# hzxie/RMNet

Hardware: AMD Instinct MI355X
Metric: frames/sec at 480p, 1 object, T=5 memory; memory-read HBM GB/s vs peak (higher is better)
Workload: dtype f32 convs; memory read = fp16 operands (K, V, q, P rounded to 11 bits), fp32 accumulate (RMNET_BANK_F16): the frame loop's default for clips with one object -- on one-object 480x854 clips whose masks HAVE a boundary (tests/live_fixture.py) mask IoU vs the CPU path 0.99993-0.99997 and foreground logi

## Files before the change

### include/rmnet_hip.h

```cpp
#ifndef RMNET_HIP_H_
#define RMNET_HIP_H_

#include <stddef.h>
#include <stdint.h>

#ifdef __cplusplus
extern "C" {
#endif

#define RMNET_ABI_VERSION 6

enum {
  RMNET_OK = 0,
  RMNET_E_INVALID_ARG = -1,
  RMNET_E_WORKSPACE = -2,
  RMNET_E_LAUNCH = -3,
  RMNET_E_UNSUPPORTED = -4
};

int rmnet_abi_version(void);
const char *rmnet_error_string(int code);

size_t rmnet_region_map_workspace_bytes(int B, int K, int H, int W);
int rmnet_region_map_f32(const float *mask, int B, int K, int H, int W, float prob_threshold,
                         int n_pts_threshold, int n_bbox_loose_pixels, float *att_map,
                         int32_t *bboxes, int32_t *cell_rects, int pad_l, int pad_t,
                         int cell_stride, int cells_h, int cells_w, void *workspace,
                         size_t workspace_bytes, void *stream);

int rmnet_region_map_warped_f32(const float *mask, const float *flow, int B, int K, int H, int W,
                                float prob_threshold, int n_pts_threshold, int n_bbox_loose_pixels,
                                float *att_map, int32_t *bboxes, int32_t *cell_rects, int pad_l,
                                int pad_t, int cell_stride, int cells_h, int cells_w, float *warped,
                                void *workspace, size_t workspace_bytes, void *stream);

int rmnet_boxes_to_cell_rects_i32(const int32_t *bboxes, int n_boxes, int k_per_batch, int pad_l,
                                  int pad_t, int cell_stride, int cells_h, int cells_w,
                                  int32_t *cell_rects, void *stream);

#define RMNET_MR_DEFAULT 0
#define RMNET_MR_FORCE_GENERIC 1
#define RMNET_MR_EXACT_FP32 2
#define RMNET_MR_F16 4
#define RMNET_BANK_F16 4
#define RMNET_MR_QX 8
#define RMNET_BANK_QX 8

size_t rmnet_memory_read_workspace_bytes(int no, int De, int Do, int T, int h, int w, int flags);
int rmnet_memory_read_f32(const float *m_key, const float *m_val, const float *q_key,
                          const float *q_val, int no, int De, int Do, int T, int h, int w,
                          long long m_chan_stride, long long m_obj_stride, long long v_chan_stride,
                          long long v_obj_stride, float *mem_val, float *p_out,
                          const int32_t *mem_rects, const int32_t *qry_rects, int flags,
                          void *workspace, size_t workspace_bytes, void *stream);

int rmnet_memory_read_f32_ev(const float *m_key, const float *m_val, const float *q_key,
                             const float *q_val, int no, int De, int Do, int T, int h, int w,
                             long long m_chan_stride, long long m_obj_stride,
                             long long v_chan_stride, long long v_obj_stride, float *mem_val,
                             float *p_out, const int32_t *mem_rects, const int32_t *qry_rects,
                             int flags, void *workspace, size_t workspace_bytes, void *stream,
                             void *ev_start, void *ev_mid, void *ev_end);

size_t rmnet_bank_bytes(int no, int Tcap, int h, int w);
size_t rmnet_bank_overflow_offset(int no, int Tcap, int h, int w);
size_t rmnet_bank_area_offset(int no, int Tcap, int h, int w);
int rmnet_bank_append_f32(void *bank, int no, int Tcap, int h, int w, int slot, const float *k4,
                          const float *v4, const int32_t *rects, void *stream);
int rmnet_bank_append_f32_at(void *bank, int no, int Tcap, int h, int w, int slot, const int32_t *slot_dev,
                             const float *k4, const float *v4, const int32_t *rects, void *stream);
int rmnet_bank_read_f32_at(void *bank, int no, int Tcap, int h, int w, int T, const int32_t *T_dev, int flags,
                           const float *q_key, const float *q_val, const int32_t *qry_rects,
                           float *mem_val, void *workspace, size_t workspace_bytes, void *stream,
                           void *ev_start, void *ev_mid, void *ev_end);
size_t rmnet_bank_read_workspace_bytes(int no, int h, int w);
size_t rmnet_bank_read_workspace_bytes_for(int no, int h, int w, int T);
int rmnet_bank_read_f32(void *bank, int no, int Tcap, int h, int w, int T,
                        const float *q_key, const float *q_val, const int32_t *qry_rects,
                        float *mem_val, void *workspace, size_t workspace_bytes, void *stream,
                        void *ev_start, void *ev_mid, void *ev_end);

int rmnet_rect_mask_f32(const float *x, int n, int C, int T, int h, int w, const int32_t *rects,
                        float *y, void *stream);

int rmnet_channel_affine_f32(const float *x, const float *scale, const float *shift,
                             const float *res, const float *res_scale, const float *res_shift,
                             int relu, long long N, int C, long long HW, float *out, void *stream);

int rmnet_affine_relu_maxpool_f32(const float *x, const float *scale, const float *shift, long long N,
                                  int C, int H, int W, float *out, void *stream);

int rmnet_upsample2x_add_f32(const float *x, const float *skip, long long N, int C, int h, int w,
                             float *out, void *stream);

int rmnet_channel_affine_nhwc_f32(const float *x, const float *scale, const float *shift, const float *res, const float *res_scale,
                                  const float *res_shift, int relu, long long rows, int C, float *out, void *stream);
int rmnet_upsample2x_add_nhwc_f32(const float *x, const float *skip, long long N, int C, int h, int w, float *out, void *stream);
int rmnet_affine_relu_maxpool_nhwc_f32(const float *x, const float *scale, const float *shift, long long N, int C, int H, int W,
                                       float *out, void *stream);

#define RMNET_CONV_RELU_IN 1
#define RMNET_CONV_RELU_OUT 2
int rmnet_conv3x3_split_f32(const float *x, const void *wpack, const float *w_unscale, const float *bias, const float *res, int flags,
                            int N, int H, int W, int Cin, float *out, int32_t *range_word, void *stream);

int rmnet_conv_split_f32(const float *x, const void *wpack, const float *w_unscale, const float *shift, const float *res, int flags,
                         int N, int H, int W, int Cin, int Cout, int ksize, int stride, float *out, float *out2, int out_split,
                         int32_t *range_word, void *stream);

#define RMNET_CONV_X_SPLIT 4
#define RMNET_CONV_OUT_SPLIT 8
int rmnet_conv_split_pre_f32(const void *x, const void *wpack, const float *w_unscale, const float *shift, const float *res, int flags,
                             int N, int H, int W, int Cin, int Cout, int ksize, int stride, void *out, float *out2, int out_split,
                             int32_t *range_word, void *stream);
int rmnet_split_act_f32(const float *x, long long M, int C, int relu, void *out, int32_t *range_word, void *stream);

int rmnet_stem_split_f32(const float *frame, const float *mask, const float *other, const void *wpack, const float *w_unscale,
                         const float *shift, int N, int H, int W, float *out, int32_t *range_word, void *stream);

int rmnet_pred_head_f32(const float *x, const float *w, const float *bias, int n, int Hq, int Wq, int C, float *out, void *stream);

#define RMNET_FLOW_RELU 1
#define RMNET_FLOW_LEAKY 2
#define RMNET_FLOW_TRANSPOSED 4
int rmnet_flow_conv_f32(const float *x, int x_ld, const void *wpack, const float *w_unscale, const float *shift, int flags, int N, int H,
                        int W, int Cin, int Cout, int ksize, int stride, float *out, int out_ld, int coff, int32_t *range_word,
                        void *stream);

size_t rmnet_flow_head_workspace_bytes(int N, int H, int W, int Cin);
int rmnet_flow_head_f32(const float *x, int x_ld, const float *wpack, const float *bias, int N, int H, int W, int Cin, float *out,
                        void *workspace, size_t workspace_bytes, void *stream);

int rmnet_flow_up_f32(const float *flow, const float *w, int N, int h, int w_, float *out, int out_ld, int coff, void *stream);

int rmnet_soft_aggregate_f32(const float *dec, const int32_t *obj_begin, int B, int K, int Hp, int Wp,
                             int pad_l, int pad_t, int H, int W, float *logit, float *prob,
                             void *stream);

int rmnet_flow_affine_f32(const float *flow, const float *m1, const float *m2, int H, int W,
                          float *out, void *stream);
size_t rmnet_flow_affine_workspace_bytes(int H, int W);
int rmnet_flow_affine_f32_host(const float *flow_host, const float *m1_host, const float *m2_host,
                               int H, int W, float *out_host, void *workspace,
                               size_t workspace_bytes, void *stream);

#ifdef __cplusplus
}
#endif
#endif
```

### rmnet_amd/_lib.py

```python

import ctypes
import os

_HERE = os.path.dirname(os.path.abspath(__file__))
LIB_PATH = os.environ.get('RMNET_HIP_LIB') or os.path.join(_HERE, 'librmnet_hip.so')

c_f32p = ctypes.c_void_p
c_i32p = ctypes.c_void_p

SIGNATURES = {
    'rmnet_abi_version': (ctypes.c_int, []),
    'rmnet_error_string': (ctypes.c_char_p, [ctypes.c_int]),
    'rmnet_region_map_workspace_bytes': (ctypes.c_size_t, [ctypes.c_int] * 4),
    'rmnet_region_map_f32': (ctypes.c_int, [
        c_f32p, ctypes.c_int, ctypes.c_int, ctypes.c_int, ctypes.c_int, ctypes.c_float, ctypes.c_int,
        ctypes.c_int, c_f32p, c_i32p, c_i32p, ctypes.c_int, ctypes.c_int, ctypes.c_int, ctypes.c_int,
        ctypes.c_int, ctypes.c_void_p, ctypes.c_size_t, ctypes.c_void_p]),
    'rmnet_region_map_warped_f32': (ctypes.c_int, [
        c_f32p, c_f32p, ctypes.c_int, ctypes.c_int, ctypes.c_int, ctypes.c_int, ctypes.c_float, ctypes.c_int,
        ctypes.c_int, c_f32p, c_i32p, c_i32p, ctypes.c_int, ctypes.c_int, ctypes.c_int, ctypes.c_int,
        ctypes.c_int, c_f32p, ctypes.c_void_p, ctypes.c_size_t, ctypes.c_void_p]),
    'rmnet_boxes_to_cell_rects_i32': (ctypes.c_int, [
        c_i32p, ctypes.c_int, ctypes.c_int, ctypes.c_int, ctypes.c_int, ctypes.c_int, ctypes.c_int,
        ctypes.c_int, c_i32p, ctypes.c_void_p]),
    'rmnet_memory_read_workspace_bytes': (ctypes.c_size_t, [ctypes.c_int] * 7),
    'rmnet_memory_read_f32': (ctypes.c_int, [
        c_f32p, c_f32p, c_f32p, c_f32p, ctypes.c_int, ctypes.c_int, ctypes.c_int, ctypes.c_int,
        ctypes.c_int, ctypes.c_int, ctypes.c_longlong, ctypes.c_longlong, ctypes.c_longlong,
        ctypes.c_longlong, c_f32p, c_f32p, c_i32p, c_i32p, ctypes.c_int, ctypes.c_void_p,
        ctypes.c_size_t, ctypes.c_void_p]),
    'rmnet_memory_read_f32_ev': (ctypes.c_int, [
        c_f32p, c_f32p, c_f32p, c_f32p, ctypes.c_int, ctypes.c_int, ctypes.c_int, ctypes.c_int,
        ctypes.c_int, ctypes.c_int, ctypes.c_longlong, ctypes.c_longlong, ctypes.c_longlong,
        ctypes.c_longlong, c_f32p, c_f32p, c_i32p, c_i32p, ctypes.c_int, ctypes.c_void_p,
        ctypes.c_size_t, ctypes.c_void_p, ctypes.c_void_p, ctypes.c_void_p, ctypes.c_void_p]),
    'rmnet_bank_bytes': (ctypes.c_size_t, [ctypes.c_int] * 4),
    'rmnet_bank_overflow_offset': (ctypes.c_size_t, [ctypes.c_int] * 4),
    'rmnet_bank_area_offset': (ctypes.c_size_t, [ctypes.c_int] * 4),
    'rmnet_bank_append_f32': (ctypes.c_int, [
        ctypes.c_void_p, ctypes.c_int, ctypes.c_int, ctypes.c_int, ctypes.c_int, ctypes.c_int, c_f32p,
        c_f32p, c_i32p, ctypes.c_void_p]),
    'rmnet_bank_append_f32_at': (ctypes.c_int, [
        ctypes.c_void_p, ctypes.c_int, ctypes.c_int, ctypes.c_int, ctypes.c_int, ctypes.c_int, c_i32p, c_f32p,
        c_f32p, c_i32p, ctypes.c_void_p]),
    'rmnet_bank_read_f32_at': (ctypes.c_int, [
        ctypes.c_void_p, ctypes.c_int, ctypes.c_int, ctypes.c_int, ctypes.c_int, ctypes.c_int, c_i32p, ctypes.c_int, c_f32p,
        c_f32p, c_i32p, c_f32p, ctypes.c_void_p, ctypes.c_size_t, ctypes.c_void_p, ctypes.c_void_p,
        ctypes.c_void_p, ctypes.c_void_p]),
    'rmnet_bank_read_workspace_bytes': (ctypes.c_size_t, [ctypes.c_int] * 3),
    'rmnet_bank_read_workspace_bytes_for': (ctypes.c_size_t, [ctypes.c_int] * 4),
    'rmnet_bank_read_f32': (ctypes.c_int, [
        ctypes.c_void_p, ctypes.c_int, ctypes.c_int, ctypes.c_int, ctypes.c_int, ctypes.c_int, c_f32p,
        c_f32p, c_i32p, c_f32p, ctypes.c_void_p, ctypes.c_size_t, ctypes.c_void_p, ctypes.c_void_p,
        ctypes.c_void_p, ctypes.c_void_p]),
    'rmnet_rect_mask_f32': (ctypes.c_int, [
        c_f32p, ctypes.c_int, ctypes.c_int, ctypes.c_int, ctypes.c_int, ctypes.c_int, c_i32p, c_f32p,
        ctypes.c_void_p]),
    'rmnet_channel_affine_f32': (ctypes.c_int, [
        c_f32p, c_f32p, c_f32p, c_f32p, c_f32p, c_f32p, ctypes.c_int, ctypes.c_longlong, ctypes.c_int,
        ctypes.c_longlong, c_f32p, ctypes.c_void_p]),
    'rmnet_upsample2x_add_f32': (ctypes.c_int, [
        c_f32p, c_f32p, ctypes.c_longlong, ctypes.c_int, ctypes.c_int, ctypes.c_int, c_f32p, ctypes.c_void_p]),
    'rmnet_soft_aggregate_f32': (ctypes.c_int, [
        c_f32p, c_i32p, ctypes.c_int, ctypes.c_int, ctypes.c_int, ctypes.c_int, ctypes.c_int, ctypes.c_int,
        ctypes.c_int, ctypes.c_int, c_f32p, c_f32p, ctypes.c_void_p]),
    'rmnet_affine_relu_maxpool_f32': (ctypes.c_int, [
        c_f32p, c_f32p, c_f32p, ctypes.c_longlong, ctypes.c_int, ctypes.c_int, ctypes.c_int, c_f32p,
        ctypes.c_void_p]),
    'rmnet_channel_affine_nhwc_f32': (ctypes.c_int, [
        c_f32p, c_f32p, c_f32p, c_f32p, c_f32p, c_f32p, ctypes.c_int, ctypes.c_longlong, ctypes.c_int, c_f32p, ctypes.c_void_p]),
    'rmnet_upsample2x_add_nhwc_f32': (ctypes.c_int, [
        c_f32p, c_f32p, ctypes.c_longlong, ctypes.c_int, ctypes.c_int, ctypes.c_int, c_f32p, ctypes.c_void_p]),
    'rmnet_affine_relu_maxpool_nhwc_f32': (ctypes.c_int, [
        c_f32p, c_f32p, c_f32p, ctypes.c_longlong, ctypes.c_int, ctypes.c_int, ctypes.c_int, c_f32p, ctypes.c_void_p]),
    'rmnet_conv3x3_split_f32': (ctypes.c_int, [
        c_f32p, ctypes.c_void_p, c_f32p, c_f32p, c_f32p, ctypes.c_int, ctypes.c_int, ctypes.c_int, ctypes.c_int, ctypes.c_int,
        c_f32p, c_i32p, ctypes.c_void_p]),
    'rmnet_conv_split_f32': (ctypes.c_int, [
        c_f32p, ctypes.c_void_p, c_f32p, c_f32p, c_f32p, ctypes.c_int, ctypes.c_int, ctypes.c_int, ctypes.c_int, ctypes.c_int,
        ctypes.c_int, ctypes.c_int, ctypes.c_int, c_f32p, c_f32p, ctypes.c_int, c_i32p, ctypes.c_void_p]),
    'rmnet_conv_split_pre_f32': (ctypes.c_int, [
        ctypes.c_void_p, ctypes.c_void_p, c_f32p, c_f32p, c_f32p, ctypes.c_int, ctypes.c_int, ctypes.c_int, ctypes.c_int, ctypes.c_int,
        ctypes.c_int, ctypes.c_int, ctypes.c_int, ctypes.c_void_p, c_f32p, ctypes.c_int, c_i32p, ctypes.c_void_p]),
    'rmnet_split_act_f32': (ctypes.c_int, [
        c_f32p, ctypes.c_longlong, ctypes.c_int, ctypes.c_int, ctypes.c_void_p, c_i32p, ctypes.c_void_p]),
    'rmnet_stem_split_f32': (ctypes.c_int, [
        c_f32p, c_f32p, c_f32p, ctypes.c_void_p, c_f32p, c_f32p, ctypes.c_int, ctypes.c_int, ctypes.c_int, c_f32p, c_i32p,
        ctypes.c_void_p]),
    'rmnet_pred_head_f32': (ctypes.c_int, [
        c_f32p, c_f32p, c_f32p, ctypes.c_int, ctypes.c_int, ctypes.c_int, ctypes.c_int, c_f32p, ctypes.c_void_p]),
    'rmnet_flow_conv_f32': (ctypes.c_int, [
        c_f32p, ctypes.c_int, ctypes.c_void_p, c_f32p, c_f32p, ctypes.c_int, ctypes.c_int, ctypes.c_int, ctypes.c_int, ctypes.c_int,
        ctypes.c_int, ctypes.c_int, ctypes.c_int, c_f32p, ctypes.c_int, ctypes.c_int, c_i32p, ctypes.c_void_p]),
    'rmnet_flow_head_workspace_bytes': (ctypes.c_size_t, [ctypes.c_int] * 4),
    'rmnet_flow_head_f32': (ctypes.c_int, [
        c_f32p, ctypes.c_int, c_f32p, c_f32p, ctypes.c_int, ctypes.c_int, ctypes.c_int, ctypes.c_int, c_f32p, ctypes.c_void_p,
        ctypes.c_size_t, ctypes.c_void_p]),
    'rmnet_flow_up_f32': (ctypes.c_int, [
        c_f32p, c_f32p, ctypes.c_int, ctypes.c_int, ctypes.c_int, c_f32p, ctypes.c_int, ctypes.c_int, ctypes.c_void_p]),
    'rmnet_flow_affine_f32': (ctypes.c_int, [
        c_f32p, c_f32p, c_f32p, ctypes.c_int, ctypes.c_int, c_f32p, ctypes.c_void_p]),
    'rmnet_flow_affine_workspace_bytes': (ctypes.c_size_t, [ctypes.c_int, ctypes.c_int]),
    'rmnet_flow_affine_f32_host': (ctypes.c_int, [
        ctypes.c_void_p, ctypes.c_void_p, ctypes.c_void_p, ctypes.c_int, ctypes.c_int,
        ctypes.c_void_p, ctypes.c_void_p, ctypes.c_size_t, ctypes.c_void_p]),
}

ABI_VERSION = 6
_lib = None


class RMNetHipError(RuntimeError):
    pass


def load():
    global _lib
    if _lib is not None:
        return _lib
    if not os.path.exists(LIB_PATH):
        raise RMNetHipError(
            'librmnet_hip.so is missing (%s). The HIP kernels are the only implementation of this '
            'path; build them with `python -m rmnet_amd.build`.' % LIB_PATH)
    lib = ctypes.CDLL(LIB_PATH)
    for name, (res, args) in SIGNATURES.items():
        fn = getattr(lib, name)
        fn.restype = res
        fn.argtypes = args
    if lib.rmnet_abi_version() != ABI_VERSION:
        raise RMNetHipError('librmnet_hip.so ABI %d != expected %d' % (lib.rmnet_abi_version(), ABI_VERSION))
    _lib = lib
    return lib


def check(code, what):
    if code != 0:
        msg = load().rmnet_error_string(code).decode()
        raise RMNetHipError('%s failed: %s (code %d)' % (what, msg, code))
```

### rmnet_amd/csrc/conv3x3.hip

```cpp
#include "common.h"

namespace rmnet {
namespace {

typedef _Float16 half8 __attribute__((ext_vector_type(8)));
typedef _Float16 half4 __attribute__((ext_vector_type(4)));
typedef float f32x4 __attribute__((ext_vector_type(4)));
typedef unsigned int u32x4 __attribute__((ext_vector_type(4)));

constexpr int kCout = 256;
constexpr int kMT = 128;
constexpr int kKT = 32;
constexpr int kThreads = 512;
constexpr float kActScale = 64.0f;
constexpr float kActUnscale = 1.0f / 64.0f;
constexpr float kF16Max = 65504.0f;
constexpr int kXPlane = kMT * kKT;
constexpr int kWPlane = kCout * kKT;
constexpr int kBufHalves = 2 * kXPlane + 2 * kWPlane;
static_assert(2 * kBufHalves * 2 <= kLdsBytesPerCU, "LDS budget");

__device__ inline int swz(int row, int chunk) { return row * kKT + ((chunk ^ ((row >> 1) & 3)) << 3); }

template <bool B>
// ... 69 lines not shown
    _Float16* xl = buf + kXPlane;
#pragma unroll
    for (int i = 0; i < 2; ++i) {
      half4 hi, lo;
#pragma unroll
      for (int e = 0; e < 4; ++e) {
        float v = in[i] ? xr[i][e] : 0.0f;
        if constexpr (decltype(relu)::value) v = v < 0.0f ? 0.0f : v;
        const float y = v * kActScale;
        if constexpr (decltype(centre)::value) bad += !(fabsf(y) <= kF16Max) ? 1 : 0;
        const float c = fminf(fmaxf(y, -kF16Max), kF16Max);
        const _Float16 h = (_Float16)c;
        hi[e] = h;
        lo[e] = (_Float16)(c - (float)h);
      }
      const int p = (tid >> 3) + 64 * i;
      const int o = swz(p, c4 >> 1) + 4 * (c4 & 1);
      *reinterpret_cast<half4*>(xh + o) = hi;
      *reinterpret_cast<half4*>(xl + o) = lo;
    }
  };
  auto store_w = [&](_Float16* buf) {
    _Float16* wb = buf + 2 * kXPlane;
#pragma unroll
    for (int i = 0; i < 4; ++i) {
      const int q = tid + kThreads * i;
      const int plane = q >> 10, co = (q >> 2) & (kCout - 1), ch = q & 3;
      *reinterpret_cast<u32x4*>(wb + plane * kWPlane + swz(co, ch)) = wr[i];
    }
  };

  f32x4 acc[4][4], accx[4][4];
#pragma unroll
  for (int i = 0; i < 4; ++i)
#pragma unroll
    for (int j = 0; j < 4; ++j) acc[i][j] = accx[i][j] = f32x4{0.f, 0.f, 0.f, 0.f};

  set_tap(0);
  load();
  if (a.relu_in)
    store_x(Flag<true>{}, Flag<false>{}, lds);
  else
    store_x(Flag<false>{}, Flag<false>{}, lds);
  store_w(lds);
  __syncthreads();
  const int fr = lane & 15, fc = lane >> 4;
  auto mma = [&](const _Float16* __restrict__ cur, auto&& halfway) __attribute__((always_inline)) {
    const _Float16* xh = cur;
    const _Float16* xl = cur + kXPlane;
    const _Float16* wh = cur + 2 * kXPlane;
    const _Float16* wl = wh + kWPlane;
    half8 bh[4], bl[4];
#pragma unroll
    for (int i = 0; i < 4; ++i) {
      const int o = swz(wm * 64 + i * 16 + fr, fc);
      bh[i] = *reinterpret_cast<const half8*>(xh + o);
      bl[i] = *reinterpret_cast<const half8*>(xl + o);
    }
#pragma unroll
    for (int j = 0; j < 4; ++j) {
      const int o = swz(wn * 64 + j * 16 + fr, fc);
      const half8 ah = *reinterpret_cast<const half8*>(wh + o);
      const half8 al = *reinterpret_cast<const half8*>(wl + o);
#pragma unroll
      for (int i = 0; i < 4; ++i) acc[i][j] = __builtin_amdgcn_mfma_f32_16x16x32_f16(ah, bh[i], acc[i][j], 0, 0, 0);
#pragma unroll
      for (int i = 0; i < 4; ++i) accx[i][j] = __builtin_amdgcn_mfma_f32_16x16x32_f16(ah, bl[i], accx[i][j], 0, 0, 0);
#pragma unroll
      for (int i = 0; i < 4; ++i) accx[i][j] = __builtin_amdgcn_mfma_f32_16x16x32_f16(al, bh[i], accx[i][j], 0, 0, 0);
      if (j == 1) halfway();
    }
  };
  int par = 0;
  auto run_taps = [&](auto relu, auto centre, int t0, int t1) __attribute__((always_inline)) {
#pragma unroll 1
    for (int tap = t0; tap < t1; ++tap) {
      if (tap) set_tap(tap);
      const int n = tap ? CB : CB - 1;
      for (int k = 0; k < n; ++k) {
        _Float16* nxt = lds + (par ^ 1) * kBufHalves;
        load();
        __builtin_amdgcn_sched_barrier(0);
        mma(lds + par * kBufHalves, [&] {
          __builtin_amdgcn_sched_barrier(0);
          store_x(relu, centre, nxt);
        });
#pragma unroll
        for (int g = 0; g < 24; ++g) {
          __builtin_amdgcn_sched_group_barrier(0x008, 1, 0);
          __builtin_amdgcn_sched_group_barrier(0x002, 3, 0);
        }
        __builtin_amdgcn_sched_barrier(0);
        store_w(nxt);
        __syncthreads();
        par ^= 1;
      }
    }
  };
  auto run = [&](auto relu) __attribute__((always_inline)) {
    run_taps(relu, Flag<false>{}, 0, 4);
    run_taps(relu, Flag<true>{}, 4, 5);
    run_taps(relu, Flag<false>{}, 5, 9);
  };
  if (a.relu_in)
    run(Flag<true>{});
  else
    run(Flag<false>{});
  mma(lds + par * kBufHalves, [] {});

  f32x4 r[4][4];
  if (a.res) {
#pragma unroll
    for (int i = 0; i < 4; ++i) {
      const int m = m0 + wm * 64 + i * 16 + fr;
#pragma unroll
      for (int j = 0; j < 4; ++j) {
        const int co = wn * 64 + j * 16 + 4 * fc;
        r[i][j] = m < a.M ? *reinterpret_cast<const f32x4*>(a.res + (size_t)m * kCout + co) : f32x4{0.f, 0.f, 0.f, 0.f};
      }
    }
  }
#pragma unroll
  for (int j = 0; j < 4; ++j) {
    const int co = wn * 64 + j * 16 + 4 * fc;
    const f32x4 us = *reinterpret_cast<const f32x4*>(a.w_unscale + co) * kActUnscale;
    const f32x4 b = a.bias ? *reinterpret_cast<const f32x4*>(a.bias + co) : f32x4{0.f, 0.f, 0.f, 0.f};
#pragma unroll
    for (int i = 0; i < 4; ++i) acc[i][j] = (acc[i][j] + accx[i][j]) * us + b;
  }
#pragma unroll
  for (int j = 0; j < 4; ++j)
#pragma unroll
    for (int i = 0; i < 4; ++i) asm volatile("" : "+v"(acc[i][j]));
#pragma unroll
  for (int j = 0; j < 4; ++j) {
    const int co = wn * 64 + j * 16 + 4 * fc;
#pragma unroll
    for (int i = 0; i < 4; ++i) {
      const int m = m0 + wm * 64 + i * 16 + fr;
      if (m >= a.M) continue;
      const size_t off = (size_t)m * kCout + co;
      f32x4 v = acc[i][j];
      if (a.res) v += r[i][j];
      if (a.relu_out) {
#pragma unroll
        for (int e = 0; e < 4; ++e) v[e] = v[e] < 0.0f ? 0.0f : v[e];
      }
      *reinterpret_cast<f32x4*>(a.out + off) = v;
    }
  }
  if (a.range && bad) atomicAdd(a.range, bad);
}

}
}

extern "C" int rmnet_conv3x3_split_f32(const float* x, const void* wpack, const float* w_unscale, const float* bias,
                                       const float* res, int flags, int N, int H, int W, int Cin, float* out,
                                       int32_t* range_word, void* stream) {
  using namespace rmnet;
  if (!x || !wpack || !w_unscale || !out || N <= 0 || H <= 0 || W <= 0 || Cin <= 0) return RMNET_E_INVALID_ARG;
  if (flags & ~(RMNET_CONV_RELU_IN | RMNET_CONV_RELU_OUT)) return RMNET_E_INVALID_ARG;
  if ((reinterpret_cast<uintptr_t>(x) | reinterpret_cast<uintptr_t>(wpack) | reinterpret_cast<uintptr_t>(w_unscale) |
       reinterpret_cast<uintptr_t>(bias) | reinterpret_cast<uintptr_t>(res) | reinterpret_cast<uintptr_t>(out)) & 15)
    return RMNET_E_INVALID_ARG;
  if (Cin % kKT) return RMNET_E_UNSUPPORTED;
  const long long M = (long long)N * H * W;
  if (M * (long long)(Cin > kCout ? Cin : kCout) >= (1LL << 31)) return RMNET_E_UNSUPPORTED;
  const char* xb = reinterpret_cast<const char*>(x);
  const char* ob = reinterpret_cast<const char*>(out);
  if (ob < xb + M * Cin * sizeof(float) && xb < ob + M * kCout * sizeof(float)) return RMNET_E_INVALID_ARG;
  ConvArgs a;
  a.x = x; a.wp = reinterpret_cast<const half8*>(wpack); a.w_unscale = w_unscale; a.bias = bias; a.res = res; a.out = out;
  a.range = range_word; a.M = (int)M; a.H = H; a.W = W; a.Cin = Cin;
  a.relu_in = (flags & RMNET_CONV_RELU_IN) != 0;
  a.relu_out = (flags & RMNET_CONV_RELU_OUT) != 0;
  hipLaunchKernelGGL(conv3x3_split, dim3((unsigned)((M + kMT - 1) / kMT)), dim3(kThreads), 0, (hipStream_t)stream, a);
  return check_launch();
}
```

### rmnet_amd/ops.py

```python

import ctypes

import numpy as np
import torch

from . import _lib


MR_FORCE_GENERIC = 1
MR_EXACT_FP32 = 2
BANK_MAX_SLOTS = 2048


def _check(t, name, dtype=torch.float32):
    if not isinstance(t, torch.Tensor):
        raise RuntimeError('%s must be a torch.Tensor' % name)
    if not t.is_cuda:
        raise RuntimeError('%s must be a CUDA tensor' % name)
    if not t.is_contiguous():
        raise RuntimeError('%s must be contiguous' % name)
    if t.dtype != dtype:
        raise RuntimeError('%s must be %s, got %s' % (name, dtype, t.dtype))


def _is_cl(t):
    return t.dim() == 4 and not t.is_contiguous() and t.is_contiguous(memory_format=torch.channels_last)


def _check_act(t, name):
    if not isinstance(t, torch.Tensor) or not t.is_cuda:
        raise RuntimeError('%s must be a CUDA tensor' % name)
    if t.dtype != torch.float32:
        raise RuntimeError('%s must be torch.float32, got %s' % (name, t.dtype))
    if not (t.is_contiguous() or _is_cl(t)):
        raise RuntimeError('%s must be contiguous (NCHW) or channels-last' % name)


def _stream(dev):
    return ctypes.c_void_p(torch.cuda.current_stream(dev).cuda_stream)


def _ptr(t):
    return ctypes.c_void_p(t.data_ptr()) if t is not None else None


def _ws(nbytes, dev):
    return torch.empty(max(int(nbytes), 256), dtype=torch.uint8, device=dev)


def region_map(mask, prob_threshold=0.5, n_pts_threshold=10, n_bbox_loose_pixels=64,
               want_map=True, cell_grid=None, flow=None, want_warped=False):
    _check(mask, 'mask')
    if mask.dim() != 4:
        raise RuntimeError('mask must be [B, K, H, W]')
    if flow is not None:
        return _region_map_warped(mask, flow, prob_threshold, n_pts_threshold, n_bbox_loose_pixels,
                                  want_map, cell_grid, want_warped)
    if want_warped:
        raise RuntimeError('want_warped needs a flow')
    lib = _lib.load()
    B, K, H, W = mask.shape
    dev = mask.device
    with torch.cuda.device(dev):
        att = torch.empty_like(mask) if want_map else None
        bboxes = torch.empty(B, K, 4, dtype=torch.int32, device=dev)
        rects = torch.empty(B, K, 4, dtype=torch.int32, device=dev) if cell_grid is not None else None
        pl, pt, st, ch, cw = cell_grid if cell_grid is not None else (0, 0, 16, 1, 1)
        nb = lib.rmnet_region_map_workspace_bytes(B, K, H, W)
        ws = _ws(nb, dev)
        rc = lib.rmnet_region_map_f32(_ptr(mask), B, K, H, W, float(prob_threshold),
                                      int(n_pts_threshold), int(n_bbox_loose_pixels), _ptr(att),
                                      _ptr(bboxes), _ptr(rects), int(pl), int(pt), int(st), int(ch),
                                      int(cw), _ptr(ws), ws.numel(), _stream(dev))
    _lib.check(rc, 'rmnet_region_map_f32')
    return att, bboxes, rects


def _region_map_warped(mask, flow, prob_threshold, n_pts_threshold, n_bbox_loose_pixels, want_map,
                       cell_grid, want_warped):
    _check(flow, 'flow')
    B, K, H, W = mask.shape
    if tuple(flow.shape) != (B, 2, H, W):
        raise RuntimeError('flow must be [B, 2, H, W]')
    lib = _lib.load()
    dev = mask.device
    with torch.cuda.device(dev):
        att = torch.empty_like(mask) if want_map else None
        bboxes = torch.empty(B, K, 4, dtype=torch.int32, device=dev)
        rects = torch.empty(B, K, 4, dtype=torch.int32, device=dev) if cell_grid is not None else None
        warped = torch.zeros_like(mask) if want_warped else None
        pl, pt, st, ch, cw = cell_grid if cell_grid is not None else (0, 0, 16, 1, 1)
        nb = lib.rmnet_region_map_workspace_bytes(B, K, H, W)
        ws = _ws(nb, dev)
        rc = lib.rmnet_region_map_warped_f32(_ptr(mask), _ptr(flow), B, K, H, W, float(prob_threshold),
                                             int(n_pts_threshold), int(n_bbox_loose_pixels), _ptr(att),
                                             _ptr(bboxes), _ptr(rects), int(pl), int(pt), int(st),
                                             int(ch), int(cw), _ptr(warped), _ptr(ws), ws.numel(),
                                             _stream(dev))
    _lib.check(rc, 'rmnet_region_map_warped_f32')
    return (att, bboxes, rects, warped) if want_warped else (att, bboxes, rects)


def boxes_to_cell_rects(bboxes, pad_l, pad_t, stride, cells_h, cells_w, k_per_batch=0):
    _check(bboxes, 'bboxes', torch.int32)
    lib = _lib.load()
    dev = bboxes.device
    out = torch.empty_like(bboxes)
    with torch.cuda.device(dev):
        rc = lib.rmnet_boxes_to_cell_rects_i32(_ptr(bboxes), bboxes.numel() // 4, int(k_per_batch),
                                               int(pad_l), int(pad_t), int(stride), int(cells_h),
                                               int(cells_w), _ptr(out), _stream(dev))
    _lib.check(rc, 'rmnet_boxes_to_cell_rects_i32')
    return out


def memory_read(m_key, m_val, q_key, q_val, mem_rects=None, qry_rects=None, want_p=False, flags=0,
                T=None, out=None, events=None):
    for t, n in ((m_key, 'm_key'), (m_val, 'm_val'), (q_key, 'q_key'), (q_val, 'q_val')):
        _check(t, n)
    if m_key.dim() != 5 or m_val.dim() != 5 or q_key.dim() != 4 or q_val.dim() != 4:
        raise RuntimeError('expected m_key/m_val [no,C,T,h,w] and q_key/q_val [no,C,h,w]')
    no, De, Tcap, h, w = m_key.shape
    Do = m_val.shape[1]
    if (m_val.shape[0], m_val.shape[2], m_val.shape[3], m_val.shape[4]) != (no, Tcap, h, w) or \
            tuple(q_key.shape) != (no, De, h, w) or tuple(q_val.shape) != (no, Do, h, w):
        raise RuntimeError('memory/query shapes do not agree')
    T = Tcap if T is None else int(T)
    if not 1 <= T <= Tcap:
        raise RuntimeError('T must be in [1, %d]' % Tcap)
    if (mem_rects is None) != (qry_rects is None):
        raise RuntimeError('mem_rects and qry_rects must be given together')
    if mem_rects is not None:
        _check(mem_rects, 'mem_rects', torch.int32)
        _check(qry_rects, 'qry_rects', torch.int32)
        if mem_rects.numel() != no * T * 4 or qry_rects.numel() != no * 4:
            raise RuntimeError('mem_rects must be [no,T,4] and qry_rects [no,4]')
    lib = _lib.load()
    dev = m_key.device
    with torch.cuda.device(dev):
        if out is None:
            out = torch.empty(no, 2 * Do, h, w, dtype=torch.float32, device=dev)
        else:
            _check(out, 'out')
        p = torch.empty(no, T * h * w, h * w, dtype=torch.float32, device=dev) if want_p else None
        nb = lib.rmnet_memory_read_workspace_bytes(no, De, Do, T, h, w, int(flags))
        ws = _ws(nb, dev)
        cs = Tcap * h * w
        ev = [ctypes.c_void_p(e) if e else None for e in (events or (None, None, None))]
        rc = lib.rmnet_memory_read_f32_ev(_ptr(m_key), _ptr(m_val), _ptr(q_key), _ptr(q_val), no, De, Do,
                                          T, h, w, cs, cs * De, cs, cs * Do, _ptr(out), _ptr(p),
                                          _ptr(mem_rects), _ptr(qry_rects), int(flags), _ptr(ws),
                                          ws.numel(), _stream(dev), ev[0], ev[1], ev[2])
    _lib.check(rc, 'rmnet_memory_read_f32')
    return out, p
# ... 184 lines not shown
    def _generic_flags(self, T):
        import warnings
        nbytes = self.no * T * (self.h * self.w) ** 2 * 4
        warnings.warn('rmnet_amd: %d memorised frames exceed the fused kernels (%d): falling back to the generic path, which '
                      'materialises the affinity (%.1f GB of workspace)' % (T, BANK_MAX_SLOTS, nbytes / 1e9))
        return MR_FORCE_GENERIC


def rect_mask(x, rects):
    _check(x, 'x')
    _check(rects, 'rects', torch.int32)
    n, C, T, h, w = x.shape
    if rects.numel() != n * T * 4:
        raise RuntimeError('rects must be [n,T,4]')
    lib = _lib.load()
    y = torch.empty_like(x)
    with torch.cuda.device(x.device):
        rc = lib.rmnet_rect_mask_f32(_ptr(x), n, C, T, h, w, _ptr(rects), _ptr(y), _stream(x.device))
    _lib.check(rc, 'rmnet_rect_mask_f32')
    return y


def channel_affine(x, scale=None, shift=None, res=None, res_scale=None, res_shift=None, relu=False,
                   out=None):
    _check_act(x, 'x')
    if x.dim() != 4:
        raise RuntimeError('x must be [N,C,H,W]')
    N, C, H, W = x.shape
    cl = _is_cl(x)
    for t, n in ((scale, 'scale'), (shift, 'shift'), (res_scale, 'res_scale'), (res_shift, 'res_shift')):
        if t is not None:
            _check(t, n)
            if t.numel() != C:
                raise RuntimeError('%s must have C = %d elements' % (n, C))
    if res is not None:
        _check_act(res, 'res')
        if res.shape != x.shape:
            raise RuntimeError('res must have the shape of x')
        if cl and not res.is_contiguous(memory_format=torch.channels_last):
            res = res.contiguous(memory_format=torch.channels_last)
        elif not cl and not res.is_contiguous():
            res = res.contiguous()
    elif res_scale is not None or res_shift is not None:
        raise RuntimeError('res_scale / res_shift without res')
    if out is None:
        out = torch.empty_like(x)
    else:
        _check_act(out, 'out')
        if out.shape != x.shape or not (out.is_contiguous(memory_format=torch.channels_last) if cl else out.is_contiguous()):
            raise RuntimeError('out must have the shape and memory format of x')
    lib = _lib.load()
    with torch.cuda.device(x.device):
        if cl and C % 4 == 0:
            rc = lib.rmnet_channel_affine_nhwc_f32(_ptr(x), _ptr(scale), _ptr(shift), _ptr(res), _ptr(res_scale), _ptr(res_shift),
                                                   2 if relu == 'leaky' else (1 if relu else 0), N * H * W, C, _ptr(out), _stream(x.device))
            _lib.check(rc, 'rmnet_channel_affine_nhwc_f32')
            return out
        if cl:
            raise RuntimeError('channels-last channel_affine needs C % 4 == 0')
        rc = lib.rmnet_channel_affine_f32(_ptr(x), _ptr(scale), _ptr(shift), _ptr(res), _ptr(res_scale),
                                          _ptr(res_shift), 2 if relu == 'leaky' else (1 if relu else 0), N, C, H * W, _ptr(out),
                                          _stream(x.device))
    _lib.check(rc, 'rmnet_channel_affine_f32')
    return out


def upsample2x_add(x, skip=None, out=None):
    _check_act(x, 'x')
    if x.dim() != 4:
        raise RuntimeError('x must be [N,C,h,w]')
    N, C, h, w = x.shape
    shape = (N, C, 2 * h, 2 * w)
    cl = _is_cl(x) or (skip is not None and _is_cl(skip))
    fmt = torch.channels_last if cl else torch.contiguous_format
    if cl:
        x = x.contiguous(memory_format=torch.channels_last)
    if skip is not None:
        _check_act(skip, 'skip')
        if tuple(skip.shape) != shape:
            raise RuntimeError('skip must be [N,C,2h,2w]')
        if cl and not _is_cl(skip):
            skip = skip.contiguous(memory_format=torch.channels_last)
    if out is None or (cl and not _is_cl(out)):
        out = torch.empty(shape, dtype=x.dtype, device=x.device, memory_format=fmt)
    else:
        _check_act(out, 'out')
        if tuple(out.shape) != shape:
            raise RuntimeError('out must be [N,C,2h,2w]')
        if not cl and not out.is_contiguous():
            raise RuntimeError('out must have the memory format of x and skip (NCHW here, out is channels-last)')
    lib = _lib.load()
    with torch.cuda.device(x.device):
        if cl:
            rc = lib.rmnet_upsample2x_add_nhwc_f32(_ptr(x), _ptr(skip), N, C, h, w, _ptr(out), _stream(x.device))
            _lib.check(rc, 'rmnet_upsample2x_add_nhwc_f32')
            return out
        rc = lib.rmnet_upsample2x_add_f32(_ptr(x), _ptr(skip), N, C, h, w, _ptr(out), _stream(x.device))
    _lib.check(rc, 'rmnet_upsample2x_add_f32')
    return out


def soft_aggregate(dec, obj_begin, K, pad, want_prob=False):
    _check(dec, 'dec')
    _check(obj_begin, 'obj_begin', torch.int32)
    if dec.dim() != 4 or dec.shape[1] != 2:
        raise RuntimeError('dec must be [n,2,Hp,Wp]')
    B = obj_begin.numel() - 1
    Hp, Wp = dec.shape[2:]
    lw, uw, lh, uh = pad
    H, W = Hp - lh - uh, Wp - lw - uw
    logit = torch.empty(B, K, H, W, dtype=dec.dtype, device=dec.device)
    prob = torch.empty_like(logit) if want_prob else None
    lib = _lib.load()
    with torch.cuda.device(dec.device):
        rc = lib.rmnet_soft_aggregate_f32(_ptr(dec), _ptr(obj_begin), B, K, Hp, Wp, lw, lh, H, W,
                                          _ptr(logit), _ptr(prob), _stream(dec.device))
    _lib.check(rc, 'rmnet_soft_aggregate_f32')
    return logit, prob


CONV_COUT = 256
CONV_RELU_IN, CONV_RELU_OUT = 1, 2


@torch.no_grad()
def conv3x3_pack(weight):
    if weight.dim() != 4 or weight.shape[0] != CONV_COUT or tuple(weight.shape[2:]) != (3, 3) or weight.shape[1] % 32:
        raise RuntimeError('conv3x3_pack needs a [256, Cin, 3, 3] weight with Cin % 32 == 0, got %s' % (tuple(weight.shape),))
    if weight.dtype != torch.float32:
        raise RuntimeError('conv3x3_pack needs fp32 weights, got %s' % weight.dtype)
    w = weight.detach().contiguous()
    cin = w.shape[1]
    amax = w.abs().amax(dim=(1, 2, 3))
    _, ex = torch.frexp(amax)
    e = torch.where(amax > 0, 15 - ex, torch.zeros_like(ex))
    ws = torch.ldexp(w, e.view(-1, 1, 1, 1).to(w.dtype))
    hi = ws.half()
    lo = (ws - hi.float()).half()
    planes = torch.stack([p.reshape(CONV_COUT, cin // 32, 32, 9).permute(3, 1, 0, 2) for p in (hi, lo)], dim=2)
    unscale = torch.ldexp(torch.ones_like(amax), (-e).to(amax.dtype))
    return planes.contiguous().view(-1).view(torch.int16), unscale.contiguous()


_range_words = {}


def conv_range_word(device):
    idx = torch.device(device).index
    idx = torch.cuda.current_device() if idx is None else idx
    w = _range_words.get(idx)
    if w is None:
        w = _range_words[idx] = torch.zeros(1, dtype=torch.int32, device=torch.device('cuda', idx))
    return w


def conv3x3_split(x, wpack, w_unscale, bias=None, res=None, relu_in=False, relu_out=False, out=None, range_word=None):
    _check_act(x, 'x')
    if x.dim() != 4 or not x.is_contiguous(memory_format=torch.channels_last):
        raise RuntimeError('x must be a channels-last [N, Cin, H, W] tensor')
    N, cin, H, W = x.shape
    if cin % 32:
        raise RuntimeError('conv3x3_split needs Cin % 32 == 0, got %d' % cin)
    _check(wpack, 'wpack', torch.int16)
    if wpack.numel() != 9 * cin * CONV_COUT * 2:
        raise RuntimeError('wpack has %d elements, a Cin = %d pack has %d' % (wpack.numel(), cin, 9 * cin * CONV_COUT * 2))
    _check(w_unscale, 'w_unscale')
    shape = (N, CONV_COUT, H, W)
    for t, n in ((bias, 'bias'),):
        if t is not None:
            _check(t, n)
            if t.numel() != CONV_COUT:
                raise RuntimeError('%s must have 256 elements' % n)
    if w_unscale.numel() != CONV_COUT:
        raise RuntimeError('w_unscale must have 256 elements')
    if res is not None:
        _check_act(res, 'res')
        if tuple(res.shape) != shape or not res.is_contiguous(memory_format=torch.channels_last):
            raise RuntimeError('res must be a channels-last [N, 256, H, W] tensor')
    if out is None:
        out = torch.empty(shape, dtype=x.dtype, device=x.device, memory_format=torch.channels_last)
    else:
        _check_act(out, 'out')
        if tuple(out.shape) != shape or not out.is_contiguous(memory_format=torch.channels_last):
            raise RuntimeError('out must be a channels-last [N, 256, H, W] tensor')
    if range_word is not None:
        _check(range_word, 'range_word', torch.int32)
    for t in (wpack, w_unscale, bias, res, out, range_word):
        if t is not None and t.device != x.device:
            raise RuntimeError('conv3x3_split: every tensor must be on %s' % x.device)
    flags = (CONV_RELU_IN if relu_in else 0) | (CONV_RELU_OUT if relu_out else 0)
    lib = _lib.load()
    with torch.cuda.device(x.device):
        rc = lib.rmnet_conv3x3_split_f32(_ptr(x), _ptr(wpack), _ptr(w_unscale), _ptr(bias), _ptr(res), flags, N, H, W, cin,
                                         _ptr(out), _ptr(range_word), _stream(x.device))
    _lib.check(rc, 'rmnet_conv3x3_split_f32')
    return out


@torch.no_grad()
def conv_split_pack(weight, bn_scale=None):
    if weight.dim() != 4 or weight.shape[2] != weight.shape[3] or weight.shape[2] not in (1, 3) or weight.shape[1] % 32 \
            or weight.shape[0] % 64:
        raise RuntimeError('conv_split_pack needs a [Cout, Cin, k, k] weight with k in (1, 3), Cin % 32 == 0 and Cout % 64 == 0, '
                           'got %s' % (tuple(weight.shape),))
    if weight.dtype != torch.float32:
        raise RuntimeError('conv_split_pack needs fp32 weights, got %s' % weight.dtype)
    cout, cin, k = weight.shape[0], weight.shape[1], weight.shape[2]
    w = weight.detach().double()
    if bn_scale is not None:
        if bn_scale.numel() != cout:
            raise RuntimeError('bn_scale must have Cout = %d elements' % cout)
        w = w * bn_scale.detach().to(w.device, torch.float64).view(-1, 1, 1, 1)
    amax = w.abs().amax(dim=(1, 2, 3))
    _, ex = torch.frexp(amax)
    e = torch.where(amax > 0, 15 - ex, torch.zeros_like(ex))
    ws = torch.ldexp(w, e.view(-1, 1, 1, 1).to(w.dtype))
    hi = ws.half()
    lo = (ws - hi.double()).half()
    planes = torch.stack([p.reshape(cout, cin // 32, 32, k * k).permute(3, 1, 0, 2) for p in (hi, lo)], dim=2)
    unscale = torch.ldexp(torch.ones_like(amax), (-e).to(amax.dtype)).float()
    return planes.contiguous().view(-1).view(torch.int16), unscale.contiguous()


CONV_X_SPLIT, CONV_OUT_SPLIT = 4, 8


def is_split_act(t):
    return isinstance(t, torch.Tensor) and t.dtype == torch.float16 and t.dim() == 6 and tuple(t.shape[4:]) == (2, 32)


def _check_split_act(t, name):
    if not is_split_act(t):
        raise RuntimeError('%s must be a split activation: torch.float16 [N, H, W, C // 32, 2, 32]' % name)
    if not t.is_cuda:
        raise RuntimeError('%s must be a CUDA tensor' % name)
    if not t.is_contiguous():
        raise RuntimeError('%s must be contiguous' % name)


def split_act(x, relu=False, range_word=None):
    _check_act(x, 'x')
    if x.dim() != 4 or not x.is_contiguous(memory_format=torch.channels_last):
        raise RuntimeError('x must be a channels-last [N, C, H, W] tensor')
    N, C, H, W = x.shape
    if C % 32 or x.numel() == 0:
        raise RuntimeError('split_act needs C % 32 == 0 and a non-empty tensor, got %s' % (tuple(x.shape),))
    if range_word is not None:
        _check(range_word, 'range_word', torch.int32)
        if range_word.device != x.device:
            raise RuntimeError('split_act: every tensor must be on %s' % x.device)
    out = torch.empty((N, H, W, C // 32, 2, 32), dtype=torch.float16, device=x.device)
    lib = _lib.load()
    with torch.cuda.device(x.device):
        rc = lib.rmnet_split_act_f32(_ptr(x), N * H * W, C, 1 if relu else 0, _ptr(out), _ptr(range_word), _stream(x.device))
    _lib.check(rc, 'rmnet_split_act_f32')
    return out


def conv_split(x, wpack, w_unscale, shift=None, res=None, ksize=3, stride=1, relu_in=False, relu_out=False, out=None,
               range_word=None, split=None, out_presplit=False):
    x_split = is_split_act(x)
    if x_split:
        _check_split_act(x, 'x')
        N, H, W = x.shape[:3]
        cin = x.shape[3] * 32
        if relu_in:
            raise RuntimeError('conv_split: relu_in cannot be applied to a split activation (its producer applies it)')
    else:
        _check_act(x, 'x')
        if x.dim() != 4 or not x.is_contiguous(memory_format=torch.channels_last):
            raise RuntimeError('x must be a channels-last [N, Cin, H, W] tensor')
        N, cin, H, W = x.shape
    if ksize not in (1, 3) or stride not in (1, 2):
        raise RuntimeError('conv_split implements ksize 1 / 3 and stride 1 / 2, got %r / %r' % (ksize, stride))
    _check(w_unscale, 'w_unscale')
    cout = w_unscale.numel()
    if cin % 32 or cout % 64 or cout == 0:
        raise RuntimeError('conv_split needs Cin % 32 == 0 and Cout % 64 == 0, got %d, %d' % (cin, cout))
    _check(wpack, 'wpack', torch.int16)
    if wpack.numel() != ksize * ksize * cin * cout * 2:
        raise RuntimeError('wpack has %d elements, a %dx%d Cin = %d Cout = %d pack has %d'
                           % (wpack.numel(), ksize, ksize, cin, cout, ksize * ksize * cin * cout * 2))
    pad = ksize // 2
    shape = (N, cout, (H + 2 * pad - ksize) // stride + 1, (W + 2 * pad - ksize) // stride + 1)
    if shift is not None:
        _check(shift, 'shift')
        if shift.numel() != cout:
            raise RuntimeError('shift must have Cout = %d elements' % cout)
    if res is not None:
        _check_act(res, 'res')
        if tuple(res.shape) != shape or not res.is_contiguous(memory_format=torch.channels_last):
            raise RuntimeError('res must be a channels-last %s tensor' % (shape,))
    out2 = None
    if out_presplit:
        if split is not None or out is not None:
            raise RuntimeError('conv_split: out_presplit returns one new split activation, without split / out')
        out = torch.empty((N, shape[2], shape[3], cout // 32, 2, 32), dtype=torch.float16, device=x.device)
    elif split is not None:
        if res is not None or out is not None or not 0 < split < cout or split % 4:
            raise RuntimeError('conv_split: split must be a multiple of 4 in (0, %d), without res / out' % cout)
        out = torch.empty((N, split) + shape[2:], dtype=torch.float32, device=x.device, memory_format=torch.channels_last)
        out2 = torch.empty((N, cout - split) + shape[2:], dtype=torch.float32, device=x.device, memory_format=torch.channels_last)
    elif out is None:
        out = torch.empty(shape, dtype=torch.float32, device=x.device, memory_format=torch.channels_last)
    else:
        _check_act(out, 'out')
        if tuple(out.shape) != shape or not out.is_contiguous(memory_format=torch.channels_last):
            raise RuntimeError('out must be a channels-last %s tensor' % (shape,))
    if range_word is not None:
        _check(range_word, 'range_word', torch.int32)
    for t in (wpack, w_unscale, shift, res, out, range_word):
        if t is not None and t.device != x.device:
            raise RuntimeError('conv_split: every tensor must be on %s' % x.device)
    flags = (CONV_RELU_IN if relu_in else 0) | (CONV_RELU_OUT if relu_out else 0)
    lib = _lib.load()
    with torch.cuda.device(x.device):
        if x_split or out_presplit:
            flags |= (CONV_X_SPLIT if x_split else 0) | (CONV_OUT_SPLIT if out_presplit else 0)
            what = 'rmnet_conv_split_pre_f32'
            rc = lib.rmnet_conv_split_pre_f32(_ptr(x), _ptr(wpack), _ptr(w_unscale), _ptr(shift), _ptr(res), flags, N, H, W, cin,
                                              cout, ksize, stride, _ptr(out), _ptr(out2), split or 0, _ptr(range_word),
                                              _stream(x.device))
        else:
            what = 'rmnet_conv_split_f32'
            rc = lib.rmnet_conv_split_f32(_ptr(x), _ptr(wpack), _ptr(w_unscale), _ptr(shift), _ptr(res), flags, N, H, W, cin, cout,
                                          ksize, stride, _ptr(out), _ptr(out2), split or 0, _ptr(range_word), _stream(x.device))
    _lib.check(rc, what)
    return out if out2 is None else (out, out2)


FLOW_RELU, FLOW_LEAKY, FLOW_TRANSPOSED = 1, 2, 4
_FLOW_ACT = {None: 0, False: 0, 'none': 0, True: FLOW_RELU, 'relu': FLOW_RELU, 'leaky': FLOW_LEAKY}


def flow_conv_phase_weights(weight):
    w = weight.permute(1, 0, 2, 3)
    phases = []
    for a in (0, 1):
        for b in (0, 1):
            ky = torch.tensor([3 - a, 1 - a], device=w.device)
            kx = torch.tensor([3 - b, 1 - b], device=w.device)
            phases.append(w.index_select(2, ky).index_select(3, kx))
    return torch.stack(phases, 0)


@torch.no_grad()
def flow_conv_pack(weight, transposed=False):
    if weight.dim() != 4 or weight.shape[2] != weight.shape[3] or weight.shape[2] not in ((4,) if transposed else (3, 5)):
# ... 311 lines not shown
```

Baseline: 583.5.

## Add register-resident weight conv3x3 kernel with LDS-staged activations as default

```diff
diff --git a/include/rmnet_hip.h b/include/rmnet_hip.h
--- a/include/rmnet_hip.h
+++ b/include/rmnet_hip.h
@@ -104,6 +104,9 @@
 int rmnet_conv3x3_split_f32(const float *x, const void *wpack, const float *w_unscale, const float *bias, const float *res, int flags,
                             int N, int H, int W, int Cin, float *out, int32_t *range_word, void *stream);
 
+int rmnet_conv3x3_split_lds_f32(const float *x, const void *wpack, const float *w_unscale, const float *bias, const float *res,
+                                int flags, int N, int H, int W, int Cin, float *out, int32_t *range_word, void *stream);
+
 int rmnet_conv_split_f32(const float *x, const void *wpack, const float *w_unscale, const float *shift, const float *res, int flags,
                          int N, int H, int W, int Cin, int Cout, int ksize, int stride, float *out, float *out2, int out_split,
                          int32_t *range_word, void *stream);
diff --git a/rmnet_amd/_lib.py b/rmnet_amd/_lib.py
--- a/rmnet_amd/_lib.py
+++ b/rmnet_amd/_lib.py
@@ -76,6 +76,9 @@
     'rmnet_conv3x3_split_f32': (ctypes.c_int, [
         c_f32p, ctypes.c_void_p, c_f32p, c_f32p, c_f32p, ctypes.c_int, ctypes.c_int, ctypes.c_int, ctypes.c_int, ctypes.c_int,
         c_f32p, c_i32p, ctypes.c_void_p]),
+    'rmnet_conv3x3_split_lds_f32': (ctypes.c_int, [
+        c_f32p, ctypes.c_void_p, c_f32p, c_f32p, c_f32p, ctypes.c_int, ctypes.c_int, ctypes.c_int, ctypes.c_int, ctypes.c_int,
+        c_f32p, c_i32p, ctypes.c_void_p]),
     'rmnet_conv_split_f32': (ctypes.c_int, [
         c_f32p, ctypes.c_void_p, c_f32p, c_f32p, c_f32p, ctypes.c_int, ctypes.c_int, ctypes.c_int, ctypes.c_int, ctypes.c_int,
         ctypes.c_int, ctypes.c_int, ctypes.c_int, c_f32p, c_f32p, ctypes.c_int, c_i32p, ctypes.c_void_p]),
diff --git a/rmnet_amd/csrc/conv3x3.hip b/rmnet_amd/csrc/conv3x3.hip
--- a/rmnet_amd/csrc/conv3x3.hip
+++ b/rmnet_amd/csrc/conv3x3.hip
@@ -245,13 +245,224 @@
   if (a.range && bad) atomicAdd(a.range, bad);
 }
 
-}
-}
-
-extern "C" int rmnet_conv3x3_split_f32(const float* x, const void* wpack, const float* w_unscale, const float* bias,
-                                       const float* res, int flags, int N, int H, int W, int Cin, float* out,
-                                       int32_t* range_word, void* stream) {
-  using namespace rmnet;
+
+constexpr int kXBufHalves = 2 * kXPlane;
+
+__global__ __launch_bounds__(kThreads) void conv3x3_wreg(ConvArgs a) {
+  __shared__ __attribute__((aligned(16))) _Float16 lds[2 * kXBufHalves];
+  const int tid = threadIdx.x, lane = tid & 63, wave = tid >> 6;
+  const int fr = lane & 15, fc = lane >> 4;
+  const int m0 = blockIdx.x * kMT;
+  const int HW = a.H * a.W, CB = a.Cin / kKT;
+
+  const int c4 = tid & 7;
+  int pm[2];
+  unsigned inside[2];
+#pragma unroll
+  for (int i = 0; i < 2; ++i) {
+    const int m = m0 + (tid >> 3) + 64 * i;
+    const bool pin = m < a.M;
+    pm[i] = pin ? m : 0;
+    const int r = pm[i] % HW;
+    const int ph = r / a.W, pw = r % a.W;
+    inside[i] = 0;
+#pragma unroll
+    for (int t = 0; t < 9; ++t) {
+      const int h = ph + t / 3 - 1, w = pw + t % 3 - 1;
+      inside[i] |= (pin && h >= 0 && h < a.H && w >= 0 && w < a.W ? 1u : 0u) << t;
+    }
+  }
+  f32x4 xr[2];
+  int bad = 0;
+  const float* xb = a.x;
+  unsigned xo[2];
+  bool in[2];
+  auto set_tap = [&](int tap) {
+    const int d = (tap / 3 - 1) * a.W + (tap % 3 - 1);
+#pragma unroll
+    for (int i = 0; i < 2; ++i) {
+      in[i] = (inside[i] >> tap) & 1;
+      xo[i] = (unsigned)(pm[i] + (in[i] ? d : 0)) * a.Cin + 4 * c4;
+    }
+    xb = a.x;
+  };
+  auto load_x = [&] {
+#pragma unroll
+    for (int i = 0; i < 2; ++i) xr[i] = *reinterpret_cast<const f32x4*>(xb + xo[i]);
+    xb += kKT;
+  };
+  half8 wa[4], wb[4];
+  const half8* wsrc = a.wp;
+  const unsigned wl = (wave * 32 + fr) * 4 + fc;
+  auto load_w = [&](half8(&w)[4]) __attribute__((always_inline)) {
+#pragma unroll
+    for (int j = 0; j < 2; ++j)
+#pragma unroll
+      for (int p = 0; p < 2; ++p) w[2 * j + p] = wsrc[wl + (unsigned)(p * (kWPlane / 8) + j * 64)];
+    wsrc += 2 * kWPlane / 8;
+  };
+  auto store_x = [&](auto relu, auto centre, _Float16* buf) __attribute__((always_inline)) {
+    _Float16* xh = buf;
+    _Float16* xl = buf + kXPlane;
+#pragma unroll
+    for (int i = 0; i < 2; ++i) {
+      half4 hi, lo;
+#pragma unroll
+      for (int e = 0; e < 4; ++e) {
+        float v = in[i] ? xr[i][e] : 0.0f;
+        if constexpr (decltype(relu)::value) v = v < 0.0f ? 0.0f : v;
+        const float y = v * kActScale;
+        if constexpr (decltype(centre)::value) bad += !(fabsf(y) <= kF16Max) ? 1 : 0;
+        const float c = fminf(fmaxf(y, -kF16Max), kF16Max);
+        const _Float16 h = (_Float16)c;
+        hi[e] = h;
+        lo[e] = (_Float16)(c - (float)h);
+      }
+      const int p = (tid >> 3) + 64 * i;
+      const int o = swz(p, c4 >> 1) + 4 * (c4 & 1);
+      *reinterpret_cast<half4*>(xh + o) = hi;
+      *reinterpret_cast<half4*>(xl + o) = lo;
+    }
+  };
+
+  f32x4 acc[8][2], accx[8][2];
+#pragma unroll
+  for (int i = 0; i < 8; ++i)
+#pragma unroll
+    for (int j = 0; j < 2; ++j) acc[i][j] = accx[i][j] = f32x4{0.f, 0.f, 0.f, 0.f};
+
+  set_tap(0);
+  load_x();
+  load_w(wa);
+  if (a.relu_in)
+    store_x(Flag<true>{}, Flag<false>{}, lds);
+  else
+    store_x(Flag<false>{}, Flag<false>{}, lds);
+  __syncthreads();
+  auto mma = [&](const _Float16* __restrict__ cur, const half8(&w)[4], auto&& halfway) __attribute__((always_inline)) {
+    const _Float16* xh = cur + swz(fr, fc);
+    const _Float16* xl = xh + kXPlane;
+    half8 bh[2], bl[2];
+    bh[0] = *reinterpret_cast<const half8*>(xh);
+    bl[0] = *reinterpret_cast<const half8*>(xl);
+#pragma unroll
+    for (int i = 0; i < 8; ++i) {
+      if (i + 1 < 8) {
+        bh[(i + 1) & 1] = *reinterpret_cast<const half8*>(xh + (i + 1) * 16 * kKT);
+        bl[(i + 1) & 1] = *reinterpret_cast<const half8*>(xl + (i + 1) * 16 * kKT);
+      }
+      const half8 h = bh[i & 1], l = bl[i & 1];
+#pragma unroll
+      for (int j = 0; j < 2; ++j) acc[i][j] = __builtin_amdgcn_mfma_f32_16x16x32_f16(w[2 * j], h, acc[i][j], 0, 0, 0);
+#pragma unroll
+      for (int j = 0; j < 2; ++j) accx[i][j] = __builtin_amdgcn_mfma_f32_16x16x32_f16(w[2 * j], l, accx[i][j], 0, 0, 0);
+#pragma unroll
+      for (int j = 0; j < 2; ++j) accx[i][j] = __builtin_amdgcn_mfma_f32_16x16x32_f16(w[2 * j + 1], h, accx[i][j], 0, 0, 0);
+      if (i == 3) halfway();
+    }
+  };
+  int par = 0;
+  auto step = [&](auto relu, auto centre, const half8(&wc)[4], half8(&wn)[4]) __attribute__((always_inline)) {
+    _Float16* nxt = lds + (par ^ 1) * kXBufHalves;
+    load_x();
+    __builtin_amdgcn_sched_barrier(0);
+    load_w(wn);
+    __builtin_amdgcn_sched_barrier(0);
+    mma(lds + par * kXBufHalves, wc, [&] {
+      __builtin_amdgcn_sched_barrier(0);
+      store_x(relu, centre, nxt);
+    });
+#pragma unroll
+    for (int g = 0; g < 24; ++g) {
+      if (g % 6 == 0 && g < 18) __builtin_amdgcn_sched_group_barrier(0x100, 2, 0);
+      __builtin_amdgcn_sched_group_barrier(0x008, 1, 0);
+      __builtin_amdgcn_sched_group_barrier(0x002, 3, 0);
+    }
+    __builtin_amdgcn_sched_barrier(0);
+    __syncthreads();
+    par ^= 1;
+  };
+  auto run_taps = [&](auto relu, auto centre, int t0, int t1) __attribute__((always_inline)) {
+#pragma unroll 1
+    for (int tap = t0; tap < t1; ++tap) {
+      if (tap) set_tap(tap);
+      const int n = tap ? CB : CB - 1;
+      int k = 0;
+#pragma unroll 1
+      for (; k + 1 < n; k += 2) {
+        step(relu, centre, wa, wb);
+        step(relu, centre, wb, wa);
+      }
+      if (k < n) {
+        step(relu, centre, wa, wb);
+#pragma unroll
+        for (int f = 0; f < 4; ++f) wa[f] = wb[f];
+      }
+    }
+  };
+  auto run = [&](auto relu) __attribute__((always_inline)) {
+    run_taps(relu, Flag<false>{}, 0, 4);
+    run_taps(relu, Flag<true>{}, 4, 5);
+    run_taps(relu, Flag<false>{}, 5, 9);
+  };
+  if (a.relu_in)
+    run(Flag<true>{});
+  else
+    run(Flag<false>{});
+  mma(lds + par * kXBufHalves, wa, [] {});
+
+  f32x4 r[8][2];
+  if (a.res) {
+#pragma unroll
+    for (int i = 0; i < 8; ++i) {
+      const int m = m0 + i * 16 + fr;
+#pragma unroll
+      for (int j = 0; j < 2; ++j) {
+        const int co = wave * 32 + j * 16 + 4 * fc;
+        r[i][j] = m < a.M ? *reinterpret_cast<const f32x4*>(a.res + (size_t)m * kCout + co) : f32x4{0.f, 0.f, 0.f, 0.f};
+      }
+    }
+  }
+#pragma unroll
+  for (int j = 0; j < 2; ++j) {
+    const int co = wave * 32 + j * 16 + 4 * fc;
+    const f32x4 us = *reinterpret_cast<const f32x4*>(a.w_unscale + co) * kActUnscale;
+    const f32x4 b = a.bias ? *reinterpret_cast<const f32x4*>(a.bias + co) : f32x4{0.f, 0.f, 0.f, 0.f};
+#pragma unroll
+    for (int i = 0; i < 8; ++i) acc[i][j] = (acc[i][j] + accx[i][j]) * us + b;
+  }
+#pragma unroll
+  for (int j = 0; j < 2; ++j)
+#pragma unroll
+    for (int i = 0; i < 8; ++i) asm volatile("" : "+v"(acc[i][j]));
+#pragma unroll
+  for (int j = 0; j < 2; ++j) {
+    const int co = wave * 32 + j * 16 + 4 * fc;
+#pragma unroll
+    for (int i = 0; i < 8; ++i) {
+      const int m = m0 + i * 16 + fr;
+      if (m >= a.M) continue;
+      const size_t off = (size_t)m * kCout + co;
+      f32x4 v = acc[i][j];
+      if (a.res) v += r[i][j];
+      if (a.relu_out) {
+#pragma unroll
+        for (int e = 0; e < 4; ++e) v[e] = v[e] < 0.0f ? 0.0f : v[e];
+      }
+      *reinterpret_cast<f32x4*>(a.out + off) = v;
+    }
+  }
+  if (a.range && bad) atomicAdd(a.range, bad);
+}
+
+}
+}
+
+namespace rmnet {
+namespace {
+
+int conv3x3_launch(void (*kernel)(ConvArgs), const float* x, const void* wpack, const float* w_unscale, const float* bias,
+                   const float* res, int flags, int N, int H, int W, int Cin, float* out, int32_t* range_word, void* stream) {
   if (!x || !wpack || !w_unscale || !out || N <= 0 || H <= 0 || W <= 0 || Cin <= 0) return RMNET_E_INVALID_ARG;
   if (flags & ~(RMNET_CONV_RELU_IN | RMNET_CONV_RELU_OUT)) return RMNET_E_INVALID_ARG;
   if ((reinterpret_cast<uintptr_t>(x) | reinterpret_cast<uintptr_t>(wpack) | reinterpret_cast<uintptr_t>(w_unscale) |
@@ -268,6 +479,21 @@
   a.range = range_word; a.M = (int)M; a.H = H; a.W = W; a.Cin = Cin;
   a.relu_in = (flags & RMNET_CONV_RELU_IN) != 0;
   a.relu_out = (flags & RMNET_CONV_RELU_OUT) != 0;
-  hipLaunchKernelGGL(conv3x3_split, dim3((unsigned)((M + kMT - 1) / kMT)), dim3(kThreads), 0, (hipStream_t)stream, a);
+  hipLaunchKernelGGL(kernel, dim3((unsigned)((M + kMT - 1) / kMT)), dim3(kThreads), 0, (hipStream_t)stream, a);
   return check_launch();
 }
+
+}
+}
+
+extern "C" int rmnet_conv3x3_split_f32(const float* x, const void* wpack, const float* w_unscale, const float* bias,
+                                       const float* res, int flags, int N, int H, int W, int Cin, float* out,
+                                       int32_t* range_word, void* stream) {
+  return rmnet::conv3x3_launch(rmnet::conv3x3_wreg, x, wpack, w_unscale, bias, res, flags, N, H, W, Cin, out, range_word, stream);
+}
+
+extern "C" int rmnet_conv3x3_split_lds_f32(const float* x, const void* wpack, const float* w_unscale, const float* bias,
+                                           const float* res, int flags, int N, int H, int W, int Cin, float* out,
+                                           int32_t* range_word, void* stream) {
+  return rmnet::conv3x3_launch(rmnet::conv3x3_split, x, wpack, w_unscale, bias, res, flags, N, H, W, Cin, out, range_word, stream);
+}
diff --git a/rmnet_amd/ops.py b/rmnet_amd/ops.py
--- a/rmnet_amd/ops.py
+++ b/rmnet_amd/ops.py
@@ -1,5 +1,6 @@
 
 import ctypes
+import os
 
 import numpy as np
 import torch
@@ -490,6 +491,18 @@
     if w is None:
         w = _range_words[idx] = torch.zeros(1, dtype=torch.int32, device=torch.device('cuda', idx))
     return w
+
+
+CONV3X3_KERNEL_DEFAULT = 'wreg'
+CONV3X3_ENTRIES = {'wreg': 'rmnet_conv3x3_split_f32', 'lds': 'rmnet_conv3x3_split_lds_f32'}
+
+
+def conv3x3_entry():
+    v = os.environ.get('RMNET_CONV3X3_KERNEL')
+    v = CONV3X3_KERNEL_DEFAULT if v is None else v.strip()
+    if v not in CONV3X3_ENTRIES:
+        raise RuntimeError('RMNET_CONV3X3_KERNEL must be one of %s, got %r' % (sorted(CONV3X3_ENTRIES), v))
+    return CONV3X3_ENTRIES[v]
 
 
 def conv3x3_split(x, wpack, w_unscale, bias=None, res=None, relu_in=False, relu_out=False, out=None, range_word=None):
@@ -527,11 +540,12 @@
         if t is not None and t.device != x.device:
             raise RuntimeError('conv3x3_split: every tensor must be on %s' % x.device)
     flags = (CONV_RELU_IN if relu_in else 0) | (CONV_RELU_OUT if relu_out else 0)
+    entry = conv3x3_entry()
     lib = _lib.load()
     with torch.cuda.device(x.device):
-        rc = lib.rmnet_conv3x3_split_f32(_ptr(x), _ptr(wpack), _ptr(w_unscale), _ptr(bias), _ptr(res), flags, N, H, W, cin,
-                                         _ptr(out), _ptr(range_word), _stream(x.device))
-    _lib.check(rc, 'rmnet_conv3x3_split_f32')
+        rc = getattr(lib, entry)(_ptr(x), _ptr(wpack), _ptr(w_unscale), _ptr(bias), _ptr(res), flags, N, H, W, cin,
+                                 _ptr(out), _ptr(range_word), _stream(x.device))
+    _lib.check(rc, entry)
     return out
 
 
```

New measurement: 592.7, median of 6. 1.02x the previous value.
